# numz/ComfyUI-SeedVR2_VideoUpscaler

Measured on NVIDIA H100. Metric: upscaled frames/sec SeedVR2-3B 720p->4K, higher is better.
Workload: dtype bf16

## Files before the change

### comfyui-seedvr2_videoupscaler_b200/csrc/gemm.cu

```cuda
#include <cuda.h>
#include <cuda_runtime.h>
#include <cuda_bf16.h>
#include <stdint.h>
#include <stdio.h>
#include <stdlib.h>

#include <type_traits>

#include "ptx.cuh"
#include "svr2_internal.h"

namespace svr2 {

constexpr int BLOCK_M = 128;
constexpr int BLOCK_K = 64;
constexpr int WGMMA_K = 16;

struct GemmParams {
  int M, N, K;
  int num_m_tiles, num_n_tiles, num_k_blocks;
  int band_h;
  int group_n;
  int a_mode;
  int tiles_w, tiles_h;
  int bw, bh;
  int taps_t, taps_h, taps_w;
  int cin_blocks;
  int cin;
  int extra_blocks;
  int pad_h, pad_w;
  int stride_t;
  int H_out, W_out, T_out;
  int epi;
  int ldc;
  long long out_frame_stride;
  int out_t_pad;
  int out_dup_head;
  int shuf_c, shuf_z;
  int shuf_H, shuf_W;
  int shuf_drop;
  float out_scale;
  const __nv_bfloat16* bias;
  const float* gate;
  const __nv_bfloat16* residual;
  void* out;
  float4* stat_partial;
  int stat_slots;
  const float* rowscale;
  float2* stat2;
  int ld_stat;
  const int* run_if;
  void* out2;
// ... 65 lines not shown
  return make_uint4(o[0], o[1], o[2], o[3]);
}

__device__ __forceinline__ void conv_tile(const GemmParams& p, int m_blk, int& t_o, int& th, int& tw) {
  const int full = p.T_out * p.band_h * p.tiles_w;
  const int band = m_blk / full;
  const int r = m_blk - band * full;
  const int rows_left = p.tiles_h - band * p.band_h;
  const int rows = rows_left < p.band_h ? rows_left : p.band_h;
  const int per = rows * p.tiles_w;
  t_o = r / per;
  const int rr = r - t_o * per;
  const int trow = rr / p.tiles_w;
  th = band * p.band_h + trow;
  tw = rr - trow * p.tiles_w;
}

__device__ __forceinline__ void tile_coords(int tile, int num_m, int num_n, int g, int& m, int& n) {
  const int per_group = g * num_m;
  const int ng = tile / per_group;
  const int r = tile - ng * per_group;
  const int n0 = ng * g;
  const int gsz = (num_n - n0) < g ? (num_n - n0) : g;
  m = r / gsz;
  n = n0 + (r - m * gsz);
}

enum : int { KIND_BF16 = 0, KIND_SWIGLU = 1, KIND_F32 = 2, KIND_ROWSTAT = 3, KIND_PEXP = 4,
             KIND_QKV21 = 5, KIND_QKV10 = 6,
             KIND_BF16_RS = 7,
// ... 138 lines not shown
              tma_load_2d(sa + L::kABytes, &tmap_b, fb, kb * BLOCK_K, n0);
            }
            advance();
          }
        }
      } else {
        const int bw = p.bw, bh = p.bh, pad_h = p.pad_h, pad_w = p.pad_w, stride_t = p.stride_t;
        const int taps_t = p.taps_t, taps_h = p.taps_h, taps_w = p.taps_w, cin_blocks = p.cin_blocks, cin = p.cin;
        for (int tile = tile0; tile < num_tiles; tile += tile_step) {
          int m_blk, n_blk;
          tile_coords(tile, num_m_tiles, num_n_tiles, p.group_n, m_blk, n_blk);
          tile_start();
          int t_o, th, tw;
          conv_tile(p, m_blk, t_o, th, tw);
          const int h0 = th * bh, w0 = tw * bw;
          const int n0 = n_blk * (SWAP ? BLOCK_M : BLOCK_N);
          int kcol = 0;
          for (int kt_ = 0; kt_ < taps_t; ++kt_) {
            const int t_in = t_o * stride_t + kt_;
            for (int kh_ = 0; kh_ < taps_h; ++kh_) {
              for (int kw_ = 0; kw_ < taps_w; ++kw_) {
                for (int cb = 0; cb < cin_blocks; ++cb) {
                  uint8_t* sa; uint64_t* fb;
                  if (acquire(sa, fb)) {
                    uint8_t* s_act = SWAP ? sa + L::kABytes : sa;
                    uint8_t* s_wgt = SWAP ? sa : sa + L::kABytes;
                    if (a_mode == 1) {
                      tma_load_4d(s_act, &tmap_a, fb, cb * BLOCK_K, w0 + kw_ - pad_w, h0 + kh_ - pad_h, t_in);
                    } else {
                      tma_load_5d(s_act, &tmap_a, fb, (kw_ & 1) * cin + cb * BLOCK_K, w0 + (kw_ >> 1), kh_ & 1,
                                  h0 + (kh_ >> 1), t_in);
                    }
                    tma_load_2d(s_wgt, &tmap_b, fb, kcol, n0);
                  }
// ... 10 lines not shown
              uint8_t* s_wgt = SWAP ? sa : sa + L::kABytes;
              tma_load_4d(s_act, &tmap_a2, fb, cb * BLOCK_K, w0, h0, t_o);
              tma_load_2d(s_wgt, &tmap_b, fb, kcol, n0);
            }
            kcol += BLOCK_K;
            advance();
          }
        }
      }
    }
  } else if (warp >= 4) {
    const int wg = (warp - 4) >> 2;
    int mstage = 0;
    uint32_t mphase = 0;
    uint32_t it = 0;
    auto mainloop = [&](auto&& tail) {
      float d[BLOCK_N / 2];
#pragma unroll
      for (int i = 0; i < BLOCK_N / 2; ++i) d[i] = 0.f;
      const int nkb = p.num_k_blocks;
      const bool leader = (threadIdx.x & 127) == 0;
      int prev = -1;
      for (int kb = 0; kb < nkb; ++kb) {
        mbar_wait(&full_bar[mstage], mphase);
        const uint32_t a_addr = smem_u32(smem + mstage * L::kStageBytes);
        const uint64_t a_desc = wgmma_desc_kmajor_sw128(a_addr + wg * 64 * 128);
        const uint64_t b_desc = wgmma_desc_kmajor_sw128(a_addr + L::kABytes);
        wgmma_fence_regs(d);
        wgmma_fence();
#pragma unroll
        for (int k = 0; k < BLOCK_K / WGMMA_K; ++k)
          wgmma_ss<BLOCK_N>(d, a_desc + uint64_t(k * 2), b_desc + uint64_t(k * 2), (kb | k) != 0);
        wgmma_commit();
        wgmma_fence_regs(d);
        wgmma_wait<1>();
// ... 44 lines not shown
              x[0] += __uint_as_float(bl << 16); x[1] += __uint_as_float(bl & 0xffff0000u);
              x[2] += __uint_as_float(bl << 16); x[3] += __uint_as_float(bl & 0xffff0000u);
              x[4] += __uint_as_float(bh << 16); x[5] += __uint_as_float(bh & 0xffff0000u);
              x[6] += __uint_as_float(bh << 16); x[7] += __uint_as_float(bh & 0xffff0000u);
            }
            const int chunk = (i >> 3) * 2 + (mj >> 1);
            stmatrix_x4(tbase + row * ROW_B + ((chunk ^ (row & SWZ)) << 4), pack_bf16x2(x[0], x[1]),
                        pack_bf16x2(x[2], x[3]), pack_bf16x2(x[4], x[5]), pack_bf16x2(x[6], x[7]));
          }
        }
        mbar_arrive(tile_full);
      };
      for (int tile = tile0; tile < num_tiles; tile += tile_step, ++it) {
        int m_blk, n_blk;
        tile_coords(tile, num_m_tiles, num_n_tiles, p.group_n, m_blk, n_blk);
        mainloop([&](float (&d)[BLOCK_N / 2]) { store_tile(d, n_blk); });
      }
    } else {
      auto acc_to_smem = [&](float (&d)[BLOCK_N / 2]) {
        named_bar_sync(1, 256);
        float* acc_w = reinterpret_cast<float*>(smem);
        const int r0 = wg * 64 + ((warp & 3) << 4) + (lane >> 2);
#pragma unroll
        for (int i = 0; i < BLOCK_N / 2; i += 4) {
          const int col = (i >> 2) * 8 + 2 * (lane & 3);
          *reinterpret_cast<float2*>(acc_w + r0 * ACC_LD + col) = make_float2(d[i], d[i + 1]);
          *reinterpret_cast<float2*>(acc_w + (r0 + 8) * ACC_LD + col) = make_float2(d[i + 2], d[i + 3]);
        }
        named_bar_sync(1, 256);
      };
      constexpr bool IS_BF16 = KIND == KIND_BF16_RS;
// ... 9 lines not shown
      const int half = (warp - 4) >> 2;
      const int row = q * 32 + lane;
      const bool active = (N_COLS >= 64) || (half == 0);
      const int col_lo = (N_COLS >= 64) ? half * COLS_W : 0;
      uint8_t* slab = smem + L::kStagingOffset + (warp - 4) * 4096;
      const int n_lim = KIND == KIND_SWIGLU ? p.N / 2 : p.N;
      const float* __restrict__ gate = p.gate;
      const __nv_bfloat16* __restrict__ resid = p.residual;
      for (int tile = tile0; tile < num_tiles; tile += tile_step) {
        int m_blk, n_blk;
        tile_coords(tile, num_m_tiles, num_n_tiles, p.group_n, m_blk, n_blk);
        if (it++ > 0) {
          fence_proxy_async_smem();
          mbar_arrive(acc_free);
        }
        mainloop(acc_to_smem);
        RowDest dst = row_dest<BLOCK_N>(p, epi, m_blk, n_blk, row, N_COLS);
        const int n_base = n_blk * (KIND == KIND_SWIGLU ? BLOCK_N / 2 : BLOCK_N);

        constexpr bool kWide = (IS_BF16 || IS_PEXP) && PH_COLS == 64;
        constexpr int N_PH = kWide ? COLS_W / 64 : 1;
        uint32_t bias_pk[N_PH];
        float2 gate2[N_PH];
        if constexpr (kWide && IS_BF16) {
#pragma unroll
          for (int ph = 0; ph < N_PH; ++ph) {
            const int cn = n_base + col_lo + ph * 64 + 2 * lane;
            const bool ok = cn < p.N;
            bias_pk[ph] = ((epi & EPI_BIAS) && ok) ? *reinterpret_cast<const uint32_t*>(bias + cn) : 0u;
            gate2[ph] = ((epi & EPI_GATE) && ok) ? *reinterpret_cast<const float2*>(gate + cn) : make_float2(0.f, 0.f);
          }
// ... 815 lines not shown
    uint64_t d[5] = {(uint64_t)Cin * 2, (uint64_t)W / 2, 2, (uint64_t)H / 2, (uint64_t)T_in_total};
    uint64_t s[4] = {(uint64_t)Cin * 4, (uint64_t)W * Cin * 2, (uint64_t)W * Cin * 4, (uint64_t)H * W * Cin * 2};
    uint32_t b[5] = {BLOCK_K, (uint32_t)bw, 1, (uint32_t)bh, 1};
    rc = make_tmap_bf16(&ta, x, 5, d, s, b);
  }
  if (rc) return rc;
  CUtensorMap ta2;
  if (x2) {
    uint64_t d[4] = {(uint64_t)C2, (uint64_t)W, (uint64_t)H, (uint64_t)T_out};
    uint64_t s2[3] = {(uint64_t)C2 * 2, (uint64_t)W * C2 * 2, (uint64_t)H * W * C2 * 2};
    uint32_t b[4] = {BLOCK_K, (uint32_t)bw, (uint32_t)bh, 1};
    rc = make_tmap_bf16(&ta2, x2, 4, d, s2, b);
    if (rc) return rc;
  }
  const int K = kt * kh * kw * Cin + (x2 ? C2 : 0);
  uint64_t db[2] = {(uint64_t)K, (uint64_t)Cout}, sb[1] = {(uint64_t)K * 2};
  uint32_t bb[2] = {BLOCK_K, (uint32_t)bn};
  rc = make_tmap_bf16(&tb, w, 2, db, sb, bb);
  if (rc) return rc;
  GemmParams p{};
  p.a_mode = stride_hw == 1 ? 1 : 2;
  p.bw = bw; p.bh = bh;
  p.tiles_w = (W_out + bw - 1) / bw;
  p.tiles_h = (H_out + bh - 1) / bh;
  p.taps_t = kt; p.taps_h = kh; p.taps_w = kw;
  p.cin_blocks = Cin / 64; p.cin = Cin;
  p.extra_blocks = x2 ? C2 / 64 : 0;
  p.pad_h = p.pad_w = pad_hw;
  p.stride_t = stride_t;
  p.H_out = H_out; p.W_out = W_out; p.T_out = T_out;
  {
// ... 6 lines not shown
      if (bhn < 2) bhn = 2;
      if (bhn > H_out) bhn = H_out;
    }
    p.band_h = (kt > 1) ? (int)bhn : (H_out + bh - 1) / bh;
  }
  p.M = T_out * p.tiles_w * p.tiles_h * BLOCK_M;
  p.N = Cout; p.K = K;
  p.num_m_tiles = T_out * p.tiles_w * p.tiles_h;
  p.num_n_tiles = (Cout + bn - 1) / bn;
  p.num_k_blocks = K / BLOCK_K;
  p.epi = epi_flags & (EPI_BIAS | EPI_RESIDUAL);
  p.ldc = ldc;
  p.out_frame_stride = (long long)H_out * W_out * ldc;
  p.out_t_pad = out_t_pad;
  p.out_dup_head = out_dup_head;
  p.bias = (const __nv_bfloat16*)bias;
  p.residual = (const __nv_bfloat16*)residual;
  p.out = y;
  if (stat_slots_out) {
    if (Cout % 8 || ldc != Cout) return set_error(SVR2_ERR_ARG, "conv stats: need Cout % 8 == 0 and ldc == Cout");
    const int slots = svr2_conv_stat_slots(Cout, H_out, W_out);
    *stat_slots_out = slots;
    if (!stat_partial) return SVR2_OK;
    const int64_t need = (int64_t)T_out * slots * (Cout / 8) * 16;
    if (stat_bytes < need) return set_error(SVR2_ERR_ARG, "conv stats: stat_partial buffer too small");
    p.stat_partial = (float4*)stat_partial;
    p.stat_slots = slots;
  }
  if (swap) return launch_gemm<256, KIND_BF16, true>(ta, tb, p, (cudaStream_t)stream, x2 ? &ta2 : nullptr);
  return dispatch_gemm(bn, ta, tb, p, (cudaStream_t)stream, x2 ? &ta2 : nullptr);
// ... 36 lines not shown
```

### comfyui-seedvr2_videoupscaler_b200/csrc/vae_engine.cu

```cuda
#include <cuda_runtime.h>
#include <math.h>
#include <stdint.h>
#include <stdio.h>
#include <string.h>

#include <string>
#include <unordered_map>
#include <utility>
#include <vector>

#include "engine_internal.h"

namespace svr2 {

struct VaeState {
  void* workspace = nullptr;
  size_t workspace_bytes = 0;
  std::vector<void*> retired;
  int64_t last_launches = 0;
};

void vae_state_destroy(svr2_engine* e) {
  if (!e || !e->vae) return;
#ifndef SVR2_HOST_TEST
// ... 59 lines not shown
      free_list.erase(free_list.begin() + i);
    }
  }
  size_t alloc_top(size_t bytes) {
    bytes = align_up(bytes ? bytes : 1);
    if (high + top_used + bytes > cap) return NONE;
    top_used += bytes;
    return cap - top_used;
  }
  size_t need() const { return high + top_used; }
};

struct Act {
  size_t off = NONE, bytes = 0;
  int T = 0, H = 0, W = 0, C = 0, pad = 0;
  size_t stat_off = NONE, stat_bytes = 0;
  int slots = 0;
  size_t frame_bytes() const { return (size_t)H * W * C * 2; }
};

struct Run {
  svr2_engine* e;
  Arena A;
  char* base;
  void* stream;
  bool slicing = false, first = true;
  bool tails = true;
  std::unordered_map<std::string, size_t> state;
  int64_t launches = 0;
  int rc = SVR2_OK;
// ... 54 lines not shown
      const size_t off = A.alloc_top(bytes);
      if (off == NONE) { err(SVR2_ERR_ARG, "svr2_vae: workspace smaller than svr2_vae_workspace_bytes()"); return; }
      it = state.emplace(key, off).first;
    }
    if (tails && !dry() && ok()) {
      if (!dev_copy(P(it->second), P(y.off) + (size_t)y.T * y.frame_bytes(), bytes, stream))
        err(SVR2_ERR_CUDA, "svr2_vae: halo copy failed");
    }
  }

  Act gn(const Act& x, const std::string& p, bool silu, int pad) {
    Act y = act(x.T, x.H, x.W, x.C, pad);
    const Tensor *g = weight(p + ".weight"), *b = weight(p + ".bias");
    if (!ok()) return y;
    const int dup = pad > 0 && first;
    if (x.stat_off != NONE) {
      const size_t cb = (size_t)x.T * x.C * 2 * 4;
      const size_t coef = take(cb);
      if (!dry() && ok())
        ck(svr2_groupnorm_from_stats_bf16(P(x.off) + (size_t)x.pad * x.frame_bytes(), P(y.off), x.T, x.H * x.W, x.C, g->ptr,
                                          b->ptr, 1e-6f, silu, pad, dup, P(x.stat_off), x.slots, P(coef), stream), 2);
      give(coef, cb);
    } else {
      const size_t sb = ((size_t)svr2_groupnorm_scratch_bytes(x.T, x.H * x.W, x.C) + 7) / 8 * 8;
      const size_t scratch = take(sb);
      if (!dry() && ok())
        ck(svr2_groupnorm_bf16(P(x.off) + (size_t)x.pad * x.frame_bytes(), P(y.off), x.T, x.H * x.W, x.C, g->ptr, b->ptr,
                               1e-6f, silu, pad, dup, (double*)P(scratch), (int64_t)sb, stream), 3);
      give(scratch, sb);
    }
// ... 7 lines not shown
    if (w->rank != 5) { err(SVR2_ERR_ARG, "svr2_vae: conv weights must be passed as [Cout, kt, kh, kw, Cin]"); return Act(); }
    const int Cout = (int)w->shape[0], kt = (int)w->shape[1], kh = (int)w->shape[2], kw = (int)w->shape[3];
    if (x.pad != kt - 1 || (int)w->shape[4] != x.C) { err(SVR2_ERR_ARG, "svr2_vae: conv input halo / channels do not match the weight"); return Act(); }
    size_t x_off = x.off;
    int T_in_total = x.pad + x.T, T_out;
    if (stride_t == 2 && !first) {
      if (x.T % 2) { err(SVR2_ERR_ARG, "svr2_vae: temporal slices after the first must hold a multiple of 4 frames"); return Act(); }
      x_off += x.frame_bytes();
      T_in_total = x.pad - 1 + x.T;
      T_out = x.T / 2;
    } else {
      T_out = (x.T - 1) / stride_t + 1;
    }
    const int Ho = stride_hw == 1 ? x.H : x.H / 2, Wo = stride_hw == 1 ? x.W : x.W / 2;
    Act y = act(T_out, Ho, Wo, Cout, out_pad);
    const bool with_stats = stats && (Cout == 128 || Cout == 256 || Cout == 512);
    if (with_stats) {
      y.slots = svr2_conv_stat_slots(Cout, Ho, Wo);
      y.stat_bytes = (size_t)T_out * y.slots * (Cout / 8) * 16;
      y.stat_off = take(y.stat_bytes);
    }
    if (residual && (residual->T != T_out || residual->H != Ho || residual->W != Wo || residual->C != Cout)) {
      err(SVR2_ERR_ARG, "svr2_vae: residual shape mismatch");
      return y;
    }
    if (dry() || !ok()) return finish_conv(y, p);
    const void* res = residual ? P(residual->off) + (size_t)residual->pad * residual->frame_bytes() - (size_t)out_pad * y.frame_bytes()
                               : nullptr;
    const int epi = SVR2_EPI_BIAS | (residual ? SVR2_EPI_RESIDUAL : 0);
    const int pad_hw = (stride_hw == 1 && kh == 3) ? 1 : 0;
    const int dup = out_pad > 0 && first;
    if (with_stats) {
      int slots = 0;
      ck(svr2_conv3d_stats_bf16(P(x_off), T_in_total, x.H, x.W, x.C, w->ptr, Cout, kt, kh, kw, stride_t, stride_hw, pad_hw,
                                T_out, epi, b->ptr, res, P(y.off), out_pad, dup, Cout, P(y.stat_off), (int64_t)y.stat_bytes,
                                &slots, stream));
      if (ok() && slots != y.slots) err(SVR2_ERR_ARG, "svr2_vae: statistics slot count differs from the plan");
    } else {
      ck(svr2_conv3d_bf16(P(x_off), T_in_total, x.H, x.W, x.C, w->ptr, Cout, kt, kh, kw, stride_t, stride_hw, pad_hw, T_out,
                          epi, b->ptr, res, P(y.off), out_pad, dup, Cout, stream));
    }
    return finish_conv(y, p);
  }
  Act finish_conv(Act& y, const std::string& p) {
    halo(y, p + ":out");
    return y;
  }

  Act conv_shortcut(const Act& h, const Act& x, const std::string& p, int out_pad) {
    const Tensor *w = weight(p + "conv2+shortcut.weight"), *b = weight(p + "conv2+shortcut.bias"), *w2 = weight(p + "conv2.weight");
    if (!ok()) return Act();
    const int Cout = (int)w->shape[0], kt = (int)w2->shape[1], kh = (int)w2->shape[2], kw = (int)w2->shape[3], C2 = x.C;
    if (h.pad != kt - 1 || h.T != x.T || h.H != x.H || h.W != x.W || h.C != Cout) { err(SVR2_ERR_ARG, "svr2_vae: fused shortcut shape mismatch"); return Act(); }
    Act y = act(h.T, h.H, h.W, Cout, out_pad);
    y.slots = svr2_conv_stat_slots(Cout, h.H, h.W);
    y.stat_bytes = (size_t)h.T * y.slots * (Cout / 8) * 16;
    y.stat_off = take(y.stat_bytes);
    if (!dry() && ok()) {
      int slots = 0;
      ck(svr2_conv3d_shortcut_stats_bf16(P(h.off), h.pad + h.T, h.H, h.W, h.C, w->ptr, Cout, kt, kh, kw, h.T, b->ptr,
                                         P(x.off) + (size_t)x.pad * x.frame_bytes(), C2, P(y.off), out_pad,
                                         out_pad > 0 && first, P(y.stat_off), (int64_t)y.stat_bytes, &slots, stream));
      if (ok() && slots != y.slots) err(SVR2_ERR_ARG, "svr2_vae: statistics slot count differs from the plan");
    }
    halo(y, p + "conv2:out");
    return y;
  }

  Act resnet(Act& x, const std::string& p, int out_pad) {
// ... 97 lines not shown
    drop(x);
    return out;
  }

  Act mid(Act& x, const std::string& p) {
    Act a = resnet(x, p + "resnets.0.", 0);
    Act b = attention(a, p + "attentions.0.");
    return resnet(b, p + "resnets.1.", 0);
  }

  Act upsample(Act& x, const std::string& p, bool temporal, int keep = 0) {
    const Tensor *w = weight(p + "upscale_conv.weight"), *b = weight(p + "upscale_conv.bias");
    const int z = temporal ? 2 : 1;
    const int T_out = x.T * z - (temporal && first ? 1 : 0);
    Act y = act(T_out, 2 * x.H, 2 * x.W, x.C, 2);
    if (!dry() && ok())
      ck(svr2_upsample_shuffle_bf16(P(x.off) + (size_t)x.pad * x.frame_bytes(), x.T, x.H, x.W, x.C, w->ptr, b->ptr, temporal, first,
                                    P(y.off), 2, first, stream));
    drop(x);
    if (keep > 0 && keep < y.T) y.T = keep;
    halo(y, p + "shuffle");
    Act c = conv(y, p + "conv", 0, nullptr, 1, 1, true);
    drop(y);
    return c;
  }

  void decode_slice(const void* zin, int dt, int64_t zin_cs, int T, int h, int w, void* out, int64_t out_cs, int keep) {
    Act x = act(T, h, w, 64, 2);
    if (!dry() && ok()) ck(ncdhw_to_ndhwc_strided(zin, dt, 16, T, h, w, zin_cs, P(x.off), 64, 2, 1.0f, stream));
    halo(x, "decoder.in");
    Act c = conv(x, "decoder.conv_in", 0, nullptr, 1, 1, true);
    drop(x);
    Act m = mid(c, "decoder.mid_block.");
    char name[96];
    for (int i = 0; i < 4 && ok(); ++i) {
      for (int j = 0; j < 3; ++j) {
        snprintf(name, sizeof name, "decoder.up_blocks.%d.resnets.%d.", i, j);
        m = resnet(m, name, 0);
      }
      if (i < 3) {
        snprintf(name, sizeof name, "decoder.up_blocks.%d.upsamplers.0.", i);
        m = upsample(m, name, i < 2, i == 1 ? keep : 0);
      }
// ... 197 lines not shown
```

### comfyui-seedvr2_videoupscaler_b200/lib.py

```python
from __future__ import annotations

import ctypes
import os
from ctypes import c_float, c_int, c_int64, c_void_p, POINTER

import torch

HERE = os.path.dirname(os.path.abspath(__file__))
LIB_PATH = os.environ.get("SVR2_LIB") or os.path.join(HERE, "csrc", "libsvr2.so")

EPI_BIAS, EPI_GATE, EPI_RESIDUAL, EPI_SWIGLU, EPI_GELU, EPI_F32, EPI_SILU = 1, 2, 4, 8, 16, 32, 128
EPI_ROWSTAT, EPI_PEXP, EPI_ROWSCALE = 256, 512, 1024

class ModelDesc(ctypes.Structure):
    _fields_ = [("variant", c_int), ("dim", c_int), ("heads", c_int), ("layers", c_int), ("mm_layers", c_int),
                ("txt_in_dim", c_int), ("in_ch", c_int), ("out_ch", c_int), ("mlp_kind", c_int), ("mlp_hidden", c_int),
                ("out_norm", c_int), ("last_vid_only", c_int), ("eps", c_float), ("timestep", c_float)]


class TensorDesc(ctypes.Structure):
    _fields_ = [("name", ctypes.c_char_p), ("data", c_void_p), ("dtype", c_int), ("rank", c_int), ("shape", c_int64 * 5)]


class DitGeometryDesc(ctypes.Structure):
    _fields_ = [(n, c_int) for n in ("n_win", "total", "max_len", "n_txt_rows", "nfreq", "rope_rows", "fuse_qkv")] + \
               [(n, c_void_p) for n in ("cu_seqlens", "row_src", "row_rope", "out_row_map", "tok_dst", "tok_rope",
                                        "txt_rows", "rope_cos", "rope_sin")]
# ... 341 lines not shown
```

### comfyui-seedvr2_videoupscaler_b200/vae.py

```python
from __future__ import annotations

import os
from ctypes import c_void_p
from typing import Dict, Optional

import torch

from . import lib
from .module import EngineModule


class Act:

    def __init__(self, T, H, W, C, pad, device, buf=None):
        self.T, self.H, self.W, self.C, self.pad = T, H, W, C, pad
        self.buf = buf if buf is not None else torch.empty(pad + T, H, W, C, device=device, dtype=torch.bfloat16)
        self.stats = None

    @property
    def frame_elems(self):
        return self.H * self.W * self.C

    def body_ptr(self):
        return self.buf.data_ptr() + self.pad * self.frame_elems * 2

    @property
    def body(self):
        return self.buf[self.pad:]


class VAEOutput:
    def __init__(self, **kw):
# ... 5 lines not shown
    def __init__(self, state_dict: Dict[str, torch.Tensor], device="cuda"):
        super().__init__(device)
        lib.device_check()
        self.meta: Dict[str, tuple] = {}
        self._load(state_dict)
        self._chunk = None
        self._sliced_plans = set()
        self.split_size = None
        self.debug = None
        self.tensor_offload_device = None
        self.native = True
        self._ws_bytes: Dict[tuple, int] = {}

    def _device_state_moved(self):
        self._drop_handle()

    def _drop_handle(self):
        h = self.__dict__.get("_handle")
        if h:
            lib.engine_destroy(h)
        self.__dict__["_handle"] = None
        if "_ws_bytes" in self.__dict__:
            self._ws_bytes.clear()

    def __del__(self):
        try:
            self._drop_handle()
        except Exception:
            pass

# ... 68 lines not shown
                raise lib.Svr2Error(f"B200VideoVAE: workspace of {workspace.numel()} bytes given, {need} needed")
            ws = workspace
        else:
            sz, need = self.plan_slices(encode, T, H, W, frames=frames)
            ws = lib.workspace(need, self.device)
        dt = {torch.float32: 0, torch.bfloat16: 1, torch.float16: 2}[src.dtype]
        if encode:
            lib.call("svr2_vae_encode", self.native_handle(), lib.ptr(src), dt, T, H, W, sz, lib.ptr(out), lib.ptr(ws),
                     ws.numel(), lib.stream())
        else:
            lib.call("svr2_vae_decode_frames", self.native_handle(), lib.ptr(src), dt, T, H, W, sz,
                     4 * T - 3 if frames is None else frames, lib.ptr(out), lib.ptr(ws), ws.numel(), lib.stream())
        lib.LAUNCHES += int(lib.load().svr2_vae_last_launches(self.native_handle())) - 1
        return out

    def _conv_w(self, w, cin_pad=None, cout_pad=None):
        O, I = w.shape[:2]
        w = w.to(self.device, torch.bfloat16).permute(0, 2, 3, 4, 1)
        if cin_pad and cin_pad > I:
            w = torch.nn.functional.pad(w, (0, cin_pad - I))
        w = w.reshape(O, -1)
        if cout_pad and cout_pad > O:
            w = torch.nn.functional.pad(w, (0, 0, 0, cout_pad - O))
        return w.contiguous()

    def _vec(self, v, pad_to=None):
        v = v.to(self.device, torch.bfloat16)
        if pad_to and pad_to > v.numel():
            v = torch.nn.functional.pad(v, (0, pad_to - v.numel()))
        return v.contiguous()

    def _load(self, sd):
        sd = dict(sd)
# ... 18 lines not shown
                W[k] = self._conv_w(v)
            elif k.endswith(".weight") and v.ndim == 4:
                raise NotImplementedError("2-D VAE checkpoints are not supported by the engine")
            else:
                W[k] = self._vec(v) if v.ndim == 1 else v.to(self.device, torch.bfloat16).contiguous()
            if k.endswith(".weight") and v.ndim == 5:
                self.meta[k + ".k"] = tuple(v.shape[2:])
                self.meta[k + ".real"] = (v.shape[0], v.shape[1])

        for k in [k for k in W if k.endswith("conv_shortcut.weight")]:
            p = k[: -len("conv_shortcut.weight")]
            wsc = W[k].reshape(W[k].shape[0], -1)
            W[p + "conv2+shortcut.weight"] = torch.cat([W[p + "conv2.weight"], wsc], 1).contiguous()
            W[p + "conv2+shortcut.bias"] = (W[p + "conv2.bias"].float() + W[p + "conv_shortcut.bias"].float()
                                            ).to(torch.bfloat16).contiguous()
        self.W = self._register("w", W)

    @property
    def _first(self) -> bool:
        return self._chunk is None or self._chunk["first"]

    def _halo(self, y: Act, key: str) -> None:
        c = self._chunk
        if c is None or y.pad == 0:
            return
        if not c["first"]:
            y.buf[: y.pad].copy_(c["state"][key])
        c["state"][key] = y.buf[-y.pad:].clone()

    def _gn(self, x: Act, prefix: str, silu: bool, pad: int) -> Act:
        y = Act(x.T, x.H, x.W, x.C, pad, self.device)
        if x.stats is not None:
            part, slots = x.stats
            coef = torch.empty(x.T * x.C * 2, device=self.device, dtype=torch.float32)
            lib.call("svr2_groupnorm_from_stats_bf16", c_void_p(x.body_ptr()), lib.ptr(y.buf), x.T, x.H * x.W, x.C,
                     lib.ptr(self.W[prefix + ".weight"]), lib.ptr(self.W[prefix + ".bias"]), 1e-6, int(silu), pad,
                     int(pad > 0 and self._first), lib.ptr(part), slots, lib.ptr(coef), lib.stream(),
                     nbytes=4.0 * x.T * x.H * x.W * x.C)
            self._halo(y, prefix)
            return y
        need = lib.load().svr2_groupnorm_scratch_bytes(x.T, x.H * x.W, x.C)
        stats = torch.empty((need + 7) // 8, device=self.device, dtype=torch.float64)
        lib.call("svr2_groupnorm_bf16", c_void_p(x.body_ptr()), lib.ptr(y.buf), x.T, x.H * x.W, x.C,
                 lib.ptr(self.W[prefix + ".weight"]), lib.ptr(self.W[prefix + ".bias"]), 1e-6, int(silu), pad,
                 int(pad > 0 and self._first), lib.ptr(stats), stats.numel() * 8, lib.stream(),
                 nbytes=6.0 * x.T * x.H * x.W * x.C)
# ... 1 lines not shown
        return y

    def _conv(self, x: Act, prefix: str, *, out_pad=0, residual: Optional[Act] = None, stride_t=1, stride_hw=1,
              stats=False) -> Act:
        w = self.W[prefix + ".weight"]
        kt, kh, kw = self.meta[prefix + ".weight.k"]
        assert x.pad == kt - 1, f"{prefix}: conv with kt={kt} needs a {kt - 1}-frame halo, got {x.pad}"
        x_ptr, T_in_total = lib.ptr(x.buf), x.pad + x.T
        if stride_t == 2 and not self._first:
            assert x.T % 2 == 0, "temporal slices after the first must hold a multiple of 4 frames"
            x_ptr, T_in_total = c_void_p(x.buf.data_ptr() + x.frame_elems * 2), x.pad - 1 + x.T
            T_out = x.T // 2
        else:
            T_out = (x.T - 1) // stride_t + 1
        Ho, Wo = (x.H, x.W) if stride_hw == 1 else (x.H // 2, x.W // 2)
        y = Act(T_out, Ho, Wo, w.shape[0], out_pad, self.device)
        res_ptr = None
        if residual is not None:
            assert (residual.T, residual.H, residual.W, residual.C) == (T_out, Ho, Wo, w.shape[0])
            res_ptr = c_void_p(residual.body_ptr() - out_pad * y.frame_elems * 2)
        epi = lib.EPI_BIAS | (lib.EPI_RESIDUAL if residual is not None else 0)
        pad_hw = 1 if (stride_hw == 1 and kh == 3) else 0
        args = (x_ptr, T_in_total, x.H, x.W, x.C, lib.ptr(w), w.shape[0], kt, kh, kw, stride_t, stride_hw,
                pad_hw, T_out, epi, lib.ptr(self.W[prefix + ".bias"]), res_ptr, lib.ptr(y.buf), out_pad,
                int(out_pad > 0 and self._first), w.shape[0])
        name, extra = "svr2_conv3d_bf16", ()
        if stats and w.shape[0] in (128, 256, 512):
            import ctypes
            slots = ctypes.c_int(lib.load().svr2_conv_stat_slots(w.shape[0], Ho, Wo))
            part = torch.empty(T_out * slots.value * (w.shape[0] // 8) * 4, device=self.device, dtype=torch.float32)
            y.stats = (part, slots.value)
            name, extra = "svr2_conv3d_stats_bf16", (lib.ptr(part), part.numel() * 4, ctypes.byref(slots))
        lib.call(name, *args, *extra, lib.stream(),
                 flops=2.0 * T_out * Ho * Wo * self.meta[prefix + ".weight.real"][0] * kt * kh * kw
                 * self.meta[prefix + ".weight.real"][1],
                 tag=(f"|{x.C}>{w.shape[0]}|k{kt}{kh}{kw}|s{stride_t}{stride_hw}|{T_out}x{Ho}x{Wo}"
                      if (lib.PROFILER is not None and lib.PROFILER.detail) else ""))
        self._halo(y, prefix + ":out")
        return y

    def _resnet(self, x: Act, p: str, out_pad=0) -> Act:
        h = self._gn(x, p + "norm1", True, 2)
        h = self._conv(h, p + "conv1", stats=True)
        h = self._gn(h, p + "norm2", True, 2)
        if (p + "conv_shortcut.weight") in self.W:
            return self._conv_shortcut(h, x, p, out_pad)
        return self._conv(h, p + "conv2", out_pad=out_pad, residual=x, stats=True)

    def _conv_shortcut(self, h: Act, x: Act, p: str, out_pad: int) -> Act:
        import ctypes
        w, b = self.W[p + "conv2+shortcut.weight"], self.W[p + "conv2+shortcut.bias"]
        kt, kh, kw = self.meta[p + "conv2.weight.k"]
        Cout, C2 = w.shape[0], x.C
        assert h.pad == kt - 1 and (h.T, h.H, h.W) == (x.T, x.H, x.W) and h.C == Cout
        y = Act(h.T, h.H, h.W, Cout, out_pad, self.device)
        args = (lib.ptr(h.buf), h.pad + h.T, h.H, h.W, h.C, lib.ptr(w), Cout, kt, kh, kw, h.T, lib.ptr(b),
                c_void_p(x.body_ptr()), C2, lib.ptr(y.buf), out_pad, int(out_pad > 0 and self._first))
        slots = ctypes.c_int(lib.load().svr2_conv_stat_slots(Cout, h.H, h.W))
        part = torch.empty(h.T * slots.value * (Cout // 8) * 4, device=self.device, dtype=torch.float32)
        y.stats = (part, slots.value)
        lib.call("svr2_conv3d_shortcut_stats_bf16", *args, lib.ptr(part), part.numel() * 4, ctypes.byref(slots), lib.stream(),
                 flops=2.0 * h.T * h.H * h.W * Cout * (kt * kh * kw * h.C + C2),
                 tag=(f"|{h.C}+{C2}>{Cout}|k{kt}{kh}{kw}|s11|{h.T}x{h.H}x{h.W}"
                      if (lib.PROFILER is not None and lib.PROFILER.detail) else ""))
        self._halo(y, p + "conv2:out")
        return y

    def _attention(self, x: Act, p: str, single_pass: bool = True) -> Act:
        C, n = x.C, x.H * x.W
        dev = self.device
# ... 51 lines not shown
        out = Act(x.T, x.H, x.W, C, 0, dev)
        xb = x.body.reshape(x.T * n, C)
        lib.linear(o, self.W[p + "to_out.0.weight"], bias=self.W[p + "to_out.0.bias"], residual=xb,
                   out=out.buf.view(x.T * n, C))
        return out

    def _mid(self, x: Act, p: str) -> Act:
        x = self._resnet(x, p + "resnets.0.")
        x = self._attention(x, p + "attentions.0.")
        return self._resnet(x, p + "resnets.1.")

    def _upsample(self, x: Act, p: str, temporal: bool, keep: Optional[int] = None) -> Act:
        z = 2 if temporal else 1
        first = self._first
        T_out = x.T * z - (1 if temporal and first else 0)
        y = Act(T_out, 2 * x.H, 2 * x.W, x.C, 2, self.device)
        lib.call("svr2_upsample_shuffle_bf16", c_void_p(x.body_ptr()), x.T, x.H, x.W, x.C,
                 lib.ptr(self.W[p + "upscale_conv.weight"]), lib.ptr(self.W[p + "upscale_conv.bias"]), int(temporal),
                 int(first), lib.ptr(y.buf), 2, int(first), lib.stream(),
                 flops=2.0 * x.T * x.H * x.W * x.C * 4 * z * x.C)
        if keep is not None and keep < y.T:
            y = Act(keep, y.H, y.W, y.C, y.pad, self.device, buf=y.buf[:y.pad + keep])
        self._halo(y, p + "shuffle")
        return self._conv(y, p + "conv", stats=True)

    BYTES_PER_PIXEL_FRAME = 1500
    DEC_STATE_BYTES_PER_PIXEL = 2 * 4400
    ENC_STATE_BYTES_PER_PIXEL = 2 * 2100

    def _frames_that_fit(self, H: int, W: int, state_bytes_per_pixel: int = 0) -> int:
        free, _ = torch.cuda.mem_get_info(self.device)
        free += torch.cuda.memory_reserved(self.device) - torch.cuda.memory_allocated(self.device)
        budget = int(0.85 * free) - state_bytes_per_pixel * H * W
        return max(1, budget // (self.BYTES_PER_PIXEL_FRAME * H * W))

    @staticmethod
    def _plan(T: int, size: int):
# ... 66 lines not shown
        else:
            size = max(1, self._frames_that_fit(8 * h, 8 * w, self.DEC_STATE_BYTES_PER_PIXEL) // 4)
        if self.split_size is not None:
            size = min(size, max(1, self.split_size // 4))
        cuts = self._plan(T, size)
        out = self._run_sliced(self._decode_slice, zin, cuts, self._decoded_per_slice(cuts, F))
        if squeeze:
            out = out.squeeze(2)
        return VAEOutput(sample=out)

    def _decode_slice(self, zin: torch.Tensor, keep: int) -> torch.Tensor:
        dev = self.device
        zin = zin.contiguous()
        _, T, h, w = zin.shape
        dt = {torch.float32: 0, torch.bfloat16: 1, torch.float16: 2}[zin.dtype]
        x = Act(T, h, w, 64, 2, dev)
        lib.call("svr2_ncdhw_to_ndhwc_bf16", lib.ptr(zin), dt, 16, T, h, w, lib.ptr(x.buf), 64, 2, 1.0, lib.stream())
        self._halo(x, "decoder.in")
        x = self._conv(x, "decoder.conv_in", stats=True)
        x = self._mid(x, "decoder.mid_block.")
        for i in range(4):
            for j in range(3):
                x = self._resnet(x, f"decoder.up_blocks.{i}.resnets.{j}.")
            if i < 3:
                x = self._upsample(x, f"decoder.up_blocks.{i}.upsamplers.0.", temporal=i < 2, keep=keep if i == 1 else None)
        assert x.T == keep
        x = self._gn(x, "decoder.conv_norm_out", True, 2)
        wt = self.W["decoder.conv_out.weight"]
        npix = (x.pad + x.T) * x.H * x.W
        ldz = (npix + 3) // 4 * 4
        z = torch.empty(wt.shape[0], ldz, device=dev, dtype=torch.float32)
# ... 128 lines not shown
```

### include/svr2.h

```cpp
#ifndef SVR2_H_
#define SVR2_H_
#include <stddef.h>
#include <stdint.h>

#ifdef __cplusplus
extern "C" {
#endif

enum svr2_status {
  SVR2_OK = 0,
  SVR2_ERR_ARG = -1,
  SVR2_ERR_CUDA = -2,
  SVR2_ERR_ARCH = -3,
};

enum svr2_epilogue {
  SVR2_EPI_BIAS = 1,
  SVR2_EPI_GATE = 2,
  SVR2_EPI_RESIDUAL = 4,
  SVR2_EPI_SWIGLU = 8,
  SVR2_EPI_GELU = 16,
  SVR2_EPI_F32 = 32,
  SVR2_EPI_SILU = 128,
  SVR2_EPI_ROWSTAT = 256,
  SVR2_EPI_PEXP = 512,
  SVR2_EPI_ROWSCALE = 1024,
};

const char* svr2_last_error(void);
int svr2_version(void);
int svr2_device_check(int* sm_count, int* cc_major, int* cc_minor);

typedef struct svr2_engine svr2_t;
typedef struct svr2_model_desc {
  int variant;
  int dim, heads;
  int layers, mm_layers;
  int txt_in_dim, in_ch, out_ch;
  int mlp_kind;
  int mlp_hidden;
  int out_norm;
// ... 37 lines not shown
int svr2_vae_decode(svr2_t* engine, const void* z, int z_dtype, int T, int h, int w, int slice_frames, void* sample,
                    void* workspace, size_t workspace_bytes, void* stream);
size_t svr2_vae_decode_frames_workspace_bytes(svr2_t* engine, int T, int h, int w, int slice_frames, int frames);
int svr2_vae_decode_frames(svr2_t* engine, const void* z, int z_dtype, int T, int h, int w, int slice_frames, int frames,
                           void* sample, void* workspace, size_t workspace_bytes, void* stream);
int64_t svr2_vae_last_launches(svr2_t* engine);

int svr2_linear_bf16(const void* a, int64_t lda, const void* w, int64_t ldw, int M, int N, int K, int epi_flags,
                     const void* bias, const float* gate, const void* residual, void* out, int64_t ldc,
                     float out_scale, void* stream);

int svr2_conv3d_bf16(const void* x, int T_in_total, int H, int W, int Cin, const void* w, int Cout, int kt, int kh,
                     int kw, int stride_t, int stride_hw, int pad_hw, int T_out, int epi_flags, const void* bias,
                     const void* residual, void* y, int out_t_pad, int out_dup_head, int ldc, void* stream);

int svr2_conv3d_stats_bf16(const void* x, int T_in_total, int H, int W, int Cin, const void* w, int Cout, int kt, int kh,
                           int kw, int stride_t, int stride_hw, int pad_hw, int T_out, int epi_flags, const void* bias,
                           const void* residual, void* y, int out_t_pad, int out_dup_head, int ldc, void* stat_partial,
                           int64_t stat_bytes, int* stat_slots, void* stream);

int svr2_conv_stat_slots(int Cout, int H_out, int W_out);

int svr2_conv3d_shortcut_stats_bf16(const void* x, int T_in_total, int H, int W, int Cin, const void* w, int Cout, int kt,
                                    int kh, int kw, int T_out, const void* bias, const void* x2, int C2, void* y,
                                    int out_t_pad, int out_dup_head, void* stat_partial, int64_t stat_bytes,
                                    int* stat_slots, void* stream);

int svr2_upsample_shuffle_bf16(const void* x, int F, int H, int W, int C, const void* w, const void* bias,
                               int temporal, int drop_head, void* y, int out_t_pad, int out_dup_head, void* stream);

// ... 108 lines not shown
```

Before: 1.344.

## Fold replicated causal-pad temporal taps into pre-summed head weights for VAE convs

For kt=3 causal convolutions on the first slice, the padded head frames are copies of the first frame. The change precomputes folded weights (sums of temporal tap slices) appended as extra output rows. The conv kernel then skips the redundant temporal taps for the first one or two output frames, using a per-tile variable K-block count and an offset into the folded weight rows. This cuts GEMM work on head frames at the cost of extra weight memory, variable per-tile K loops, and some bf16 rounding of the summed weights.

```diff
diff --git a/comfyui-seedvr2_videoupscaler_b200/csrc/gemm.cu b/comfyui-seedvr2_videoupscaler_b200/csrc/gemm.cu
--- a/comfyui-seedvr2_videoupscaler_b200/csrc/gemm.cu
+++ b/comfyui-seedvr2_videoupscaler_b200/csrc/gemm.cu
@@ -36,6 +36,7 @@
   long long out_frame_stride;
   int out_t_pad;
   int out_dup_head;
+  int fold_t, fold_n;
   int shuf_c, shuf_z;
   int shuf_H, shuf_W;
   int shuf_drop;
@@ -131,6 +132,13 @@
   const int trow = rr / p.tiles_w;
   th = band * p.band_h + trow;
   tw = rr - trow * p.tiles_w;
+}
+
+__device__ __forceinline__ int conv_k_blocks(const GemmParams& p, int m_blk) {
+  if (p.fold_t == 0) return p.num_k_blocks;
+  int t_o, th, tw;
+  conv_tile(p, m_blk, t_o, th, tw);
+  return t_o < p.fold_t ? p.num_k_blocks - (p.taps_t - 1 - t_o) * p.taps_h * p.taps_w * p.cin_blocks : p.num_k_blocks;
 }
 
 __device__ __forceinline__ void tile_coords(int tile, int num_m, int num_n, int g, int& m, int& n) {
@@ -299,10 +307,15 @@
           int t_o, th, tw;
           conv_tile(p, m_blk, t_o, th, tw);
           const int h0 = th * bh, w0 = tw * bw;
-          const int n0 = n_blk * (SWAP ? BLOCK_M : BLOCK_N);
-          int kcol = 0;
-          for (int kt_ = 0; kt_ < taps_t; ++kt_) {
-            const int t_in = t_o * stride_t + kt_;
+          int n0 = n_blk * (SWAP ? BLOCK_M : BLOCK_N);
+          int taps = taps_t, kcol = 0;
+          if (t_o < p.fold_t) {
+            taps = t_o + 1;
+            kcol = t_o == 0 ? 2 * taps_h * taps_w * cin : 0;
+            n0 += p.fold_n;
+          }
+          for (int kt_ = 0; kt_ < taps; ++kt_) {
+            const int t_in = t_o * stride_t + taps_t - taps + kt_;
             for (int kh_ = 0; kh_ < taps_h; ++kh_) {
               for (int kw_ = 0; kw_ < taps_w; ++kw_) {
                 for (int cb = 0; cb < cin_blocks; ++cb) {
@@ -343,11 +356,10 @@
     int mstage = 0;
     uint32_t mphase = 0;
     uint32_t it = 0;
-    auto mainloop = [&](auto&& tail) {
+    auto mainloop = [&](int nkb, auto&& tail) {
       float d[BLOCK_N / 2];
 #pragma unroll
       for (int i = 0; i < BLOCK_N / 2; ++i) d[i] = 0.f;
-      const int nkb = p.num_k_blocks;
       const bool leader = (threadIdx.x & 127) == 0;
       int prev = -1;
       for (int kb = 0; kb < nkb; ++kb) {
@@ -422,7 +434,7 @@
       for (int tile = tile0; tile < num_tiles; tile += tile_step, ++it) {
         int m_blk, n_blk;
         tile_coords(tile, num_m_tiles, num_n_tiles, p.group_n, m_blk, n_blk);
-        mainloop([&](float (&d)[BLOCK_N / 2]) { store_tile(d, n_blk); });
+        mainloop(conv_k_blocks(p, m_blk), [&](float (&d)[BLOCK_N / 2]) { store_tile(d, n_blk); });
       }
     } else {
       auto acc_to_smem = [&](float (&d)[BLOCK_N / 2]) {
@@ -462,7 +474,7 @@
           fence_proxy_async_smem();
           mbar_arrive(acc_free);
         }
-        mainloop(acc_to_smem);
+        mainloop(conv_k_blocks(p, m_blk), acc_to_smem);
         RowDest dst = row_dest<BLOCK_N>(p, epi, m_blk, n_blk, row, N_COLS);
         const int n_base = n_blk * (KIND == KIND_SWIGLU ? BLOCK_N / 2 : BLOCK_N);
 
@@ -1308,7 +1320,10 @@
     if (rc) return rc;
   }
   const int K = kt * kh * kw * Cin + (x2 ? C2 : 0);
-  uint64_t db[2] = {(uint64_t)K, (uint64_t)Cout}, sb[1] = {(uint64_t)K * 2};
+  const bool fold = (epi_flags & SVR2_EPI_FOLD_HEAD) != 0;
+  if (fold && (kt != 3 || x2 || Cout % bn))
+    return set_error(SVR2_ERR_ARG, "svr2_conv3d_bf16: SVR2_EPI_FOLD_HEAD needs kt = 3, no shortcut and Cout a multiple of the n-tile");
+  uint64_t db[2] = {(uint64_t)K, (uint64_t)(fold ? 2 * Cout : Cout)}, sb[1] = {(uint64_t)K * 2};
   uint32_t bb[2] = {BLOCK_K, (uint32_t)bn};
   rc = make_tmap_bf16(&tb, w, 2, db, sb, bb);
   if (rc) return rc;
@@ -1345,6 +1360,10 @@
   p.out_frame_stride = (long long)H_out * W_out * ldc;
   p.out_t_pad = out_t_pad;
   p.out_dup_head = out_dup_head;
+  if (fold) {
+    p.fold_t = stride_t == 1 ? (T_out < 2 ? T_out : 2) : 1;
+    p.fold_n = Cout;
+  }
   p.bias = (const __nv_bfloat16*)bias;
   p.residual = (const __nv_bfloat16*)residual;
   p.out = y;
diff --git a/comfyui-seedvr2_videoupscaler_b200/csrc/vae_engine.cu b/comfyui-seedvr2_videoupscaler_b200/csrc/vae_engine.cu
--- a/comfyui-seedvr2_videoupscaler_b200/csrc/vae_engine.cu
+++ b/comfyui-seedvr2_videoupscaler_b200/csrc/vae_engine.cu
@@ -97,6 +97,7 @@
 struct Act {
   size_t off = NONE, bytes = 0;
   int T = 0, H = 0, W = 0, C = 0, pad = 0;
+  bool rep = false;
   size_t stat_off = NONE, stat_bytes = 0;
   int slots = 0;
   size_t frame_bytes() const { return (size_t)H * W * C * 2; }
@@ -181,6 +182,7 @@
     const Tensor *g = weight(p + ".weight"), *b = weight(p + ".bias");
     if (!ok()) return y;
     const int dup = pad > 0 && first;
+    y.rep = dup;
     if (x.stat_off != NONE) {
       const size_t cb = (size_t)x.T * x.C * 2 * 4;
       const size_t coef = take(cb);
@@ -218,6 +220,7 @@
     }
     const int Ho = stride_hw == 1 ? x.H : x.H / 2, Wo = stride_hw == 1 ? x.W : x.W / 2;
     Act y = act(T_out, Ho, Wo, Cout, out_pad);
+    y.rep = out_pad > 0 && first;
     const bool with_stats = stats && (Cout == 128 || Cout == 256 || Cout == 512);
     if (with_stats) {
       y.slots = svr2_conv_stat_slots(Cout, Ho, Wo);
@@ -228,23 +231,34 @@
       err(SVR2_ERR_ARG, "svr2_vae: residual shape mismatch");
       return y;
     }
+    const Tensor* wf = x.rep ? head_weight(p + ".weight", kt, Cout, (int64_t)kt * kh * kw * x.C) : nullptr;
     if (dry() || !ok()) return finish_conv(y, p);
     const void* res = residual ? P(residual->off) + (size_t)residual->pad * residual->frame_bytes() - (size_t)out_pad * y.frame_bytes()
                                : nullptr;
-    const int epi = SVR2_EPI_BIAS | (residual ? SVR2_EPI_RESIDUAL : 0);
+    const int epi = SVR2_EPI_BIAS | (residual ? SVR2_EPI_RESIDUAL : 0) | (wf ? SVR2_EPI_FOLD_HEAD : 0);
     const int pad_hw = (stride_hw == 1 && kh == 3) ? 1 : 0;
     const int dup = out_pad > 0 && first;
+    const void* wp = wf ? wf->ptr : w->ptr;
     if (with_stats) {
       int slots = 0;
-      ck(svr2_conv3d_stats_bf16(P(x_off), T_in_total, x.H, x.W, x.C, w->ptr, Cout, kt, kh, kw, stride_t, stride_hw, pad_hw,
+      ck(svr2_conv3d_stats_bf16(P(x_off), T_in_total, x.H, x.W, x.C, wp, Cout, kt, kh, kw, stride_t, stride_hw, pad_hw,
                                 T_out, epi, b->ptr, res, P(y.off), out_pad, dup, Cout, P(y.stat_off), (int64_t)y.stat_bytes,
                                 &slots, stream));
       if (ok() && slots != y.slots) err(SVR2_ERR_ARG, "svr2_vae: statistics slot count differs from the plan");
     } else {
-      ck(svr2_conv3d_bf16(P(x_off), T_in_total, x.H, x.W, x.C, w->ptr, Cout, kt, kh, kw, stride_t, stride_hw, pad_hw, T_out,
+      ck(svr2_conv3d_bf16(P(x_off), T_in_total, x.H, x.W, x.C, wp, Cout, kt, kh, kw, stride_t, stride_hw, pad_hw, T_out,
                           epi, b->ptr, res, P(y.off), out_pad, dup, Cout, stream));
     }
     return finish_conv(y, p);
+  }
+  const Tensor* head_weight(const std::string& name, int kt, int Cout, int64_t K) {
+    if (kt != 3 || !ok()) return nullptr;
+    const Tensor* t = find(e, name + ":head");
+    if (t && (t->rank != 2 || t->shape[0] != 2 * (int64_t)Cout || t->shape[1] != K)) {
+      err(SVR2_ERR_ARG, "svr2_vae: folded head weights must be [2 Cout, K]");
+      return nullptr;
+    }
+    return t;
   }
   Act finish_conv(Act& y, const std::string& p) {
     halo(y, p + ":out");
@@ -257,6 +271,7 @@
     const int Cout = (int)w->shape[0], kt = (int)w2->shape[1], kh = (int)w2->shape[2], kw = (int)w2->shape[3], C2 = x.C;
     if (h.pad != kt - 1 || h.T != x.T || h.H != x.H || h.W != x.W || h.C != Cout) { err(SVR2_ERR_ARG, "svr2_vae: fused shortcut shape mismatch"); return Act(); }
     Act y = act(h.T, h.H, h.W, Cout, out_pad);
+    y.rep = out_pad > 0 && first;
     y.slots = svr2_conv_stat_slots(Cout, h.H, h.W);
     y.stat_bytes = (size_t)h.T * y.slots * (Cout / 8) * 16;
     y.stat_off = take(y.stat_bytes);
@@ -384,6 +399,7 @@
     const int z = temporal ? 2 : 1;
     const int T_out = x.T * z - (temporal && first ? 1 : 0);
     Act y = act(T_out, 2 * x.H, 2 * x.W, x.C, 2);
+    y.rep = first;
     if (!dry() && ok())
       ck(svr2_upsample_shuffle_bf16(P(x.off) + (size_t)x.pad * x.frame_bytes(), x.T, x.H, x.W, x.C, w->ptr, b->ptr, temporal, first,
                                     P(y.off), 2, first, stream));
@@ -397,6 +413,7 @@
 
   void decode_slice(const void* zin, int dt, int64_t zin_cs, int T, int h, int w, void* out, int64_t out_cs, int keep) {
     Act x = act(T, h, w, 64, 2);
+    x.rep = first;
     if (!dry() && ok()) ck(ncdhw_to_ndhwc_strided(zin, dt, 16, T, h, w, zin_cs, P(x.off), 64, 2, 1.0f, stream));
     halo(x, "decoder.in");
     Act c = conv(x, "decoder.conv_in", 0, nullptr, 1, 1, true);
diff --git a/comfyui-seedvr2_videoupscaler_b200/lib.py b/comfyui-seedvr2_videoupscaler_b200/lib.py
--- a/comfyui-seedvr2_videoupscaler_b200/lib.py
+++ b/comfyui-seedvr2_videoupscaler_b200/lib.py
@@ -10,7 +10,7 @@
 LIB_PATH = os.environ.get("SVR2_LIB") or os.path.join(HERE, "csrc", "libsvr2.so")
 
 EPI_BIAS, EPI_GATE, EPI_RESIDUAL, EPI_SWIGLU, EPI_GELU, EPI_F32, EPI_SILU = 1, 2, 4, 8, 16, 32, 128
-EPI_ROWSTAT, EPI_PEXP, EPI_ROWSCALE = 256, 512, 1024
+EPI_ROWSTAT, EPI_PEXP, EPI_ROWSCALE, EPI_FOLD_HEAD = 256, 512, 1024, 2048
 
 class ModelDesc(ctypes.Structure):
     _fields_ = [("variant", c_int), ("dim", c_int), ("heads", c_int), ("layers", c_int), ("mm_layers", c_int),
diff --git a/comfyui-seedvr2_videoupscaler_b200/vae.py b/comfyui-seedvr2_videoupscaler_b200/vae.py
--- a/comfyui-seedvr2_videoupscaler_b200/vae.py
+++ b/comfyui-seedvr2_videoupscaler_b200/vae.py
@@ -12,10 +12,11 @@
 
 class Act:
 
-    def __init__(self, T, H, W, C, pad, device, buf=None):
+    def __init__(self, T, H, W, C, pad, device, buf=None, rep=False):
         self.T, self.H, self.W, self.C, self.pad = T, H, W, C, pad
         self.buf = buf if buf is not None else torch.empty(pad + T, H, W, C, device=device, dtype=torch.bfloat16)
         self.stats = None
+        self.rep = rep
 
     @property
     def frame_elems(self):
@@ -51,6 +52,10 @@
 
     def _device_state_moved(self):
         self._drop_handle()
+        W = self.__dict__.get("W")
+        for k in [k for k in W.keys() if k.endswith(":head")] if W is not None else ():
+            head = W[k]
+            self._buffers[W._names[k[: -len(":head")]]] = head[: head.shape[0] // 2]
 
     def _drop_handle(self):
         h = self.__dict__.get("_handle")
@@ -149,9 +154,9 @@
         lib.LAUNCHES += int(lib.load().svr2_vae_last_launches(self.native_handle())) - 1
         return out
 
-    def _conv_w(self, w, cin_pad=None, cout_pad=None):
+    def _conv_w(self, w, cin_pad=None, cout_pad=None, dtype=torch.bfloat16):
         O, I = w.shape[:2]
-        w = w.to(self.device, torch.bfloat16).permute(0, 2, 3, 4, 1)
+        w = w.to(self.device, dtype).permute(0, 2, 3, 4, 1)
         if cin_pad and cin_pad > I:
             w = torch.nn.functional.pad(w, (0, cin_pad - I))
         w = w.reshape(O, -1)
@@ -200,7 +205,21 @@
             W[p + "conv2+shortcut.weight"] = torch.cat([W[p + "conv2.weight"], wsc], 1).contiguous()
             W[p + "conv2+shortcut.bias"] = (W[p + "conv2.bias"].float() + W[p + "conv_shortcut.bias"].float()
                                             ).to(torch.bfloat16).contiguous()
+        for k in [k for k in W if k.endswith(".weight")]:
+            if (self.meta.get(k + ".k", (0,))[0] != 3 or k in ("encoder.conv_in.weight", "decoder.conv_out.weight")
+                    or (k.endswith("conv2.weight") and k.replace("conv2.weight", "conv_shortcut.weight") in W)):
+                continue
+            W[k + ":head"] = self._fold_head(self._conv_w(sd[k], cin_pad=64 if k == "decoder.conv_in.weight" else None,
+                                                          dtype=torch.float32))
+            W[k] = W[k + ":head"][: W[k].shape[0]]
         self.W = self._register("w", W)
+
+    @staticmethod
+    def _fold_head(w: torch.Tensor) -> torch.Tensor:
+        n = w.shape[1] // 3
+        w01, w2 = w[:, :n].float() + w[:, n:2 * n].float(), w[:, 2 * n:].float()
+        fold = torch.cat([w01, w2, w01 + w2], 1)
+        return torch.cat([w, fold], 0).to(torch.bfloat16).contiguous()
 
     @property
     def _first(self) -> bool:
@@ -215,7 +234,7 @@
         c["state"][key] = y.buf[-y.pad:].clone()
 
     def _gn(self, x: Act, prefix: str, silu: bool, pad: int) -> Act:
-        y = Act(x.T, x.H, x.W, x.C, pad, self.device)
+        y = Act(x.T, x.H, x.W, x.C, pad, self.device, rep=pad > 0 and self._first)
         if x.stats is not None:
             part, slots = x.stats
             coef = torch.empty(x.T * x.C * 2, device=self.device, dtype=torch.float32)
@@ -247,14 +266,16 @@
         else:
             T_out = (x.T - 1) // stride_t + 1
         Ho, Wo = (x.H, x.W) if stride_hw == 1 else (x.H // 2, x.W // 2)
-        y = Act(T_out, Ho, Wo, w.shape[0], out_pad, self.device)
+        y = Act(T_out, Ho, Wo, w.shape[0], out_pad, self.device, rep=out_pad > 0 and self._first)
         res_ptr = None
         if residual is not None:
             assert (residual.T, residual.H, residual.W, residual.C) == (T_out, Ho, Wo, w.shape[0])
             res_ptr = c_void_p(residual.body_ptr() - out_pad * y.frame_elems * 2)
-        epi = lib.EPI_BIAS | (lib.EPI_RESIDUAL if residual is not None else 0)
+        wf = self.W.get(prefix + ".weight:head") if (x.rep and kt == 3) else None
+        folded = 0 if wf is None else (3 if stride_t == 1 and T_out >= 2 else 2)
+        epi = lib.EPI_BIAS | (lib.EPI_RESIDUAL if residual is not None else 0) | (lib.EPI_FOLD_HEAD if wf is not None else 0)
         pad_hw = 1 if (stride_hw == 1 and kh == 3) else 0
-        args = (x_ptr, T_in_total, x.H, x.W, x.C, lib.ptr(w), w.shape[0], kt, kh, kw, stride_t, stride_hw,
+        args = (x_ptr, T_in_total, x.H, x.W, x.C, lib.ptr(w if wf is None else wf), w.shape[0], kt, kh, kw, stride_t, stride_hw,
                 pad_hw, T_out, epi, lib.ptr(self.W[prefix + ".bias"]), res_ptr, lib.ptr(y.buf), out_pad,
                 int(out_pad > 0 and self._first), w.shape[0])
         name, extra = "svr2_conv3d_bf16", ()
@@ -265,7 +286,7 @@
             y.stats = (part, slots.value)
             name, extra = "svr2_conv3d_stats_bf16", (lib.ptr(part), part.numel() * 4, ctypes.byref(slots))
         lib.call(name, *args, *extra, lib.stream(),
-                 flops=2.0 * T_out * Ho * Wo * self.meta[prefix + ".weight.real"][0] * kt * kh * kw
+                 flops=2.0 * (kt * T_out - folded) * Ho * Wo * self.meta[prefix + ".weight.real"][0] * kh * kw
                  * self.meta[prefix + ".weight.real"][1],
                  tag=(f"|{x.C}>{w.shape[0]}|k{kt}{kh}{kw}|s{stride_t}{stride_hw}|{T_out}x{Ho}x{Wo}"
                       if (lib.PROFILER is not None and lib.PROFILER.detail) else ""))
@@ -286,7 +307,7 @@
         kt, kh, kw = self.meta[p + "conv2.weight.k"]
         Cout, C2 = w.shape[0], x.C
         assert h.pad == kt - 1 and (h.T, h.H, h.W) == (x.T, x.H, x.W) and h.C == Cout
-        y = Act(h.T, h.H, h.W, Cout, out_pad, self.device)
+        y = Act(h.T, h.H, h.W, Cout, out_pad, self.device, rep=out_pad > 0 and self._first)
         args = (lib.ptr(h.buf), h.pad + h.T, h.H, h.W, h.C, lib.ptr(w), Cout, kt, kh, kw, h.T, lib.ptr(b),
                 c_void_p(x.body_ptr()), C2, lib.ptr(y.buf), out_pad, int(out_pad > 0 and self._first))
         slots = ctypes.c_int(lib.load().svr2_conv_stat_slots(Cout, h.H, h.W))
@@ -368,13 +389,13 @@
         z = 2 if temporal else 1
         first = self._first
         T_out = x.T * z - (1 if temporal and first else 0)
-        y = Act(T_out, 2 * x.H, 2 * x.W, x.C, 2, self.device)
+        y = Act(T_out, 2 * x.H, 2 * x.W, x.C, 2, self.device, rep=first)
         lib.call("svr2_upsample_shuffle_bf16", c_void_p(x.body_ptr()), x.T, x.H, x.W, x.C,
                  lib.ptr(self.W[p + "upscale_conv.weight"]), lib.ptr(self.W[p + "upscale_conv.bias"]), int(temporal),
                  int(first), lib.ptr(y.buf), 2, int(first), lib.stream(),
                  flops=2.0 * x.T * x.H * x.W * x.C * 4 * z * x.C)
         if keep is not None and keep < y.T:
-            y = Act(keep, y.H, y.W, y.C, y.pad, self.device, buf=y.buf[:y.pad + keep])
+            y = Act(keep, y.H, y.W, y.C, y.pad, self.device, buf=y.buf[:y.pad + keep], rep=y.rep)
         self._halo(y, p + "shuffle")
         return self._conv(y, p + "conv", stats=True)
 
@@ -471,7 +492,7 @@
         zin = zin.contiguous()
         _, T, h, w = zin.shape
         dt = {torch.float32: 0, torch.bfloat16: 1, torch.float16: 2}[zin.dtype]
-        x = Act(T, h, w, 64, 2, dev)
+        x = Act(T, h, w, 64, 2, dev, rep=self._first)
         lib.call("svr2_ncdhw_to_ndhwc_bf16", lib.ptr(zin), dt, 16, T, h, w, lib.ptr(x.buf), 64, 2, 1.0, lib.stream())
         self._halo(x, "decoder.in")
         x = self._conv(x, "decoder.conv_in", stats=True)
diff --git a/include/svr2.h b/include/svr2.h
--- a/include/svr2.h
+++ b/include/svr2.h
@@ -25,6 +25,7 @@
   SVR2_EPI_ROWSTAT = 256,
   SVR2_EPI_PEXP = 512,
   SVR2_EPI_ROWSCALE = 1024,
+  SVR2_EPI_FOLD_HEAD = 2048,
 };
 
 const char* svr2_last_error(void);
@@ -92,6 +93,7 @@
                      int kw, int stride_t, int stride_hw, int pad_hw, int T_out, int epi_flags, const void* bias,
                      const void* residual, void* y, int out_t_pad, int out_dup_head, int ldc, void* stream);
 
+
 int svr2_conv3d_stats_bf16(const void* x, int T_in_total, int H, int W, int Cin, const void* w, int Cout, int kt, int kh,
                            int kw, int stride_t, int stride_hw, int pad_hw, int T_out, int epi_flags, const void* bias,
                            const void* residual, void* y, int out_t_pad, int out_dup_head, int ldc, void* stat_partial,
```

Result: faster. 1.527, median of 6 (+13.6%).
